# zacz08/ADM

Hardware: AMD Instinct MI355X
Metric: train images/sec (CIFAR-10 32x32 uncond DDM UNet, 1 optimizer step/iter) + 10-step sample images/sec (higher is better)
Workload: dtype f32; 1 GPU; BASELINE configs[1]: CIFAR-10 32x32 uncond two-decoder DhariwalUNet (216M params), bs=128/GPU fp32, ddm_const schedule, dropout 0.1, loss_simple (LPIPS term needs unfetchable VGG16 weights), clip 1.0 + AdamW + EMA(every 8); global_batch=128, image=3x32x32, parallelism=dp1, valid=True

## Files before the change

adm_amd/csrc/conv_wino2d_x6.hip:

```cpp
#include "common.h"
#include "../../include/adm_hip.h"
#include <type_traits>

#ifndef X6_TL
#define X6_TL 0
#endif
#ifndef X6_SHARE
#define X6_SHARE 0
#endif
#ifndef X6_ABL
#define X6_ABL 0
#endif

namespace {

struct X6P {
  const float* x; const unsigned short* w; const float* bias; const float* res; float* y;
  int Mt, N, H, W, Hh, Wh, Cin, ldx, ldy, ldr, wrows, tilesN, xbytes, wbytes, plane;
  int splitk, chunks_per_split; float* ws;
  int ybytes, rbytes;
  int up;
  const float* amax_x; float wscale;
};

typedef __attribute__((address_space(3))) void x6_lds_void;
typedef __bf16 bf16x8 __attribute__((ext_vector_type(8)));
typedef unsigned u32x2 __attribute__((ext_vector_type(2)));
typedef unsigned u32x4 __attribute__((ext_vector_type(4)));
constexpr int X6P_T = 64, X6N = 64, X6K = 16;
[[maybe_unused]] constexpr int X6_A_STAGE = 4 * 3 * X6P_T * X6K;
[[maybe_unused]] constexpr int X6_B_STAGE = 4 * 3 * X6N * X6K;
typedef _Float16 f16x8 __attribute__((ext_vector_type(8)));
typedef _Float16 f16x2 __attribute__((ext_vector_type(2)));
template <int FMT, int NB = 2> struct X6Fmt {
  static constexpr int TERMS = FMT ? 2 : 3;
  static constexpr int NT = 32 * NB;
  static constexpr int CONS = 2 * NB;
  static constexpr int THREADS = (CONS + 4) * 64;
  static constexpr int A_STAGE = 4 * TERMS * X6P_T * X6K;
  static constexpr int B_STAGE = 4 * TERMS * NT * X6K;
  static constexpr int DMA_PER_WAVE = 2 * TERMS;
  static constexpr int RB = NB > 2 ? 3 : 4;
  static constexpr int PD = NB > 2 ? 3 : 4;
};
__device__ __host__ inline float h3_scale(float amax) {
  if (!(amax > 0.f) || !(amax < 3e38f)) return 1.f;
  int e;
  frexpf(16000.f / amax, &e);
  return ldexpf(1.f, e - 1);
}
constexpr int X6_RA = 2;

__device__ __forceinline__ void x6_barrier() {
  __builtin_amdgcn_fence(__ATOMIC_RELEASE, "workgroup", "local");
  __builtin_amdgcn_s_barrier();
// ... 50 lines not shown

__device__ __forceinline__ void x6_store(const f32x4 (&e)[4], unsigned short* la) {
  if (X6_ABL & 2) return;
  const f32x4 v[4] = {p_sub4(e[0], e[2]), p_add4(e[1], e[2]), p_sub4(e[2], e[1]), p_sub4(e[1], e[3])};
#pragma unroll
  for (int ex = 0; ex < 4; ++ex) {
    u32x2 t0, t1, t2;
    split3_pack(v[ex], t0, t1, t2);
    *reinterpret_cast<u32x2*>(la + (ex * 3 + 0) * X6P_T * X6K) = t0;
    *reinterpret_cast<u32x2*>(la + (ex * 3 + 1) * X6P_T * X6K) = t1;
    *reinterpret_cast<u32x2*>(la + (ex * 3 + 2) * X6P_T * X6K) = t2;
  }
}

#ifndef X6_KB_N
#define X6_KB_N 4
#endif
constexpr int X6_KB = X6_KB_N;
struct X6Seq {
  int k0, len, ey, cc, skip2;
  __device__ __forceinline__ void init(int chunks, int up) { k0 = 0; len = min(X6_KB, chunks); ey = 0; cc = 0; skip2 = up; }
  __device__ __forceinline__ int chunk() const { return k0 + cc; }
  __device__ __forceinline__ bool done() const { return len <= 0; }
  __device__ __forceinline__ void next(int chunks) {
    if (++cc == len) {
      cc = 0;
      ++ey;
      if (skip2 && ey == 2) ++ey;
      if (ey == 4) { ey = 0; k0 += len; len = min(X6_KB, chunks - k0); }
    }
  }
};

template <int FMT, int NB>
__global__ __launch_bounds__((2 * NB + 4) * 64) void wino2d_x6_kernel(X6P p) {
  using F = X6Fmt<FMT, NB>;
  constexpr int TERMS = F::TERMS;
  float sa = 1.f, inv_scale = 1.f;
  if (FMT) { sa = h3_scale(adm_amax_read(p.amax_x)); inv_scale = 1.f / (sa * p.wscale); }
  extern __shared__ __attribute__((aligned(16))) unsigned short smem6[];
  unsigned short* As = smem6;
  unsigned short* Bs = smem6 + X6_RA * F::A_STAGE;
  const int tid = threadIdx.x, lane = tid & 63, hw_wid = tid >> 6;
  const bool producer = hw_wid >= F::CONS;
  const int wid = producer ? hw_wid - F::CONS : hw_wid;
  int bid = blockIdx.x;
  {
    const int nwg = gridDim.x, q = nwg >> 3, r = nwg & 7, xcd = bid & 7, idx = bid >> 3;
    bid = (xcd < r ? xcd * (q + 1) : r * (q + 1) + (xcd - r) * q) + idx;
  }
  const int tilesM = gridDim.x / p.tilesN;
  const int tm = bid % tilesM, tn = bid / tilesM;
  const int mt0 = tm * X6P_T, n0 = tn * F::NT;
  constexpr unsigned OOB = 0x80000000u;

  const int c_begin = (p.splitk > 1) ? (int)blockIdx.y * p.chunks_per_split : 0;
  const int chunks = (p.splitk > 1) ? min(p.chunks_per_split, (p.Cin >> 4) - c_begin) : (p.Cin >> 4);
  const int S = (p.up ? 3 : 4) * chunks;

  if (producer) {
    const __amdgpu_buffer_rsrc_t rs_x = __builtin_amdgcn_make_buffer_rsrc(const_cast<float*>(p.x), 0, p.xbytes, 0x00020000);
    const int ptid = wid * 64 + lane;
    const int pl = ptid >> 2, aq = ptid & 3;
    unsigned a_base = 0, colmask = 0, rowmask = 0;
    bool take_l = false, take_r = false;
    {
      const int t = mt0 + pl;
      if (t < p.Mt) {
        const int xp = t % p.Wh;
        const int u = t / p.Wh;
        const int ty = u % p.Hh, b = u / p.Hh;
        a_base = p.up ? (unsigned)((((long)b * p.Hh + ty) * p.Wh + xp) * p.ldx + aq * 4) * 4u
                      : (unsigned)((((long)b * p.H + 2 * ty) * p.W + 2 * xp) * p.ldx + aq * 4) * 4u;
        colmask = (xp > 0 ? 1u : 0u) | 6u | (2 * xp + 2 < p.W ? 8u : 0u);
        rowmask = (ty > 0 ? 1u : 0u) | 6u | (2 * ty + 2 < p.H ? 8u : 0u);
        if (X6_SHARE && !p.up) {
          take_l = xp > 0 && (pl & 15) != 0;
          take_r = xp + 1 < p.Wh && (pl & 15) != 15 && t + 1 < p.Mt;
          if (take_l) colmask &= ~1u;
          if (take_r) colmask &= ~8u;
        }
      }
    }
    unsigned short* la = As + pl * X6K + ((((aq >> 1) ^ (pl >> 3)) & 1) << 3) + (aq & 1) * 4;
    X6Seq ld; ld.init(chunks, p.up);
    unsigned a_voff[2][4];
    int voff_ey = -1;
    auto set_rows = [&]() {
      const int ey = ld.ey;
      const int iA = (ey == 0) ? 0 : 1, iB = (ey == 3) ? 3 : 2;
      const bool live = !ld.done();
      const bool vA = ((rowmask >> iA) & 1u) && live, vB = ((rowmask >> iB) & 1u) && live;
      const int offA = (p.up ? ((iA + 1) >> 1) - 1 : iA - 1) * (p.up ? p.Wh : p.W) * p.ldx * 4;
      const int offB = (p.up ? ((iB + 1) >> 1) - 1 : iB - 1) * (p.up ? p.Wh : p.W) * p.ldx * 4;
#pragma unroll
      for (int j = 0; j < 4; ++j) {
// ... 20 lines not shown
      if (!ld.done()) ld.next(chunks);
    };
    auto store = [&](int d, int slot) {
      f32x4 e[4];
      if (set_ey[d] == 1) {
#pragma unroll
        for (int j = 0; j < 4; ++j) e[j] = p_add4(dA[d][j], dB[d][j]);
      } else if (set_ey[d] == 2) {
#pragma unroll
        for (int j = 0; j < 4; ++j) e[j] = p_sub4(dB[d][j], dA[d][j]);
      } else {
#pragma unroll
        for (int j = 0; j < 4; ++j) e[j] = p_sub4(dA[d][j], dB[d][j]);
      }
      if (X6_SHARE && !p.up) {
        f32x4 el, er;
#pragma unroll
        for (int i = 0; i < 4; ++i) { el[i] = __shfl_up(e[2][i], 4, 64); er[i] = __shfl_down(e[1][i], 4, 64); }
        if (take_l) e[0] = el;
        if (take_r) e[3] = er;
      }
      if (FMT) h3_store(e, la + slot * F::A_STAGE, sa);
      else x6_store(e, la + slot * F::A_STAGE);
    };
#pragma unroll
    for (int d = 0; d < D; ++d) issue(d);
    __builtin_amdgcn_sched_barrier(0);
    constexpr int TRIP = (D & 1) ? 2 * D : D;
    for (int t = 0; t < S; t += TRIP) {
#pragma unroll
      for (int k = 0; k < TRIP; ++k) {
        const int d = k % D;
        if (t + k < S) {
          const bool tl = X6_TL && p.ws && blockIdx.x == 0 && tid == F::CONS * 64 && t + k < 48;
          unsigned long long* TL = reinterpret_cast<unsigned long long*>(p.ws) + 1024 + (t + k) * 4;
          if (tl) TL[0] = __builtin_readcyclecounter();
          store(d, k & 1);
          __builtin_amdgcn_sched_barrier(0);
          if (tl) { asm volatile("s_waitcnt lgkmcnt(0)" ::: "memory"); TL[1] = __builtin_readcyclecounter(); }
          issue(d);
          __builtin_amdgcn_sched_barrier(0);
          if (tl) TL[2] = __builtin_readcyclecounter();
          x6_barrier();
          if (tl) TL[3] = __builtin_readcyclecounter();
        }
      }
    }
    return;
  }

  const __amdgpu_buffer_rsrc_t rs_w = __builtin_amdgcn_make_buffer_rsrc(const_cast<unsigned short*>(p.w), 0, p.wbytes, 0x00020000);
  const int wm = wid / NB, wn = wid % NB;
  const int lr = lane & 31, lh = lane >> 5;
  if (p.splitk > 1) {
    p.y = p.ws + (long)blockIdx.y * ((long)p.Mt * 4) * p.N;
    p.ldy = p.N; p.bias = nullptr; p.res = nullptr;
    const long sb = (long)p.Mt * 4 * p.N * 4;
    p.ybytes = sb < (1L << 31) ? (int)sb : 0;
  }
  constexpr int QW = F::DMA_PER_WAVE;
  unsigned b_voff[QW];
#pragma unroll
  for (int i = 0; i < QW; ++i) {
    const int q = wid * QW + i, pt = q / NB;
    const int row = (q % NB) * 32 + (lane >> 1);
    const int n = n0 + row;
    const int half = (lane ^ (row >> 3)) & 1;
    b_voff[i] = (n < p.wrows) ? (unsigned)((((long)pt * p.wrows + n) * 16 + half * 8) * 2) : OOB;
  }
  X6Seq lb; lb.init(chunks, p.up);
  int ld_slot = 0;
  auto issue_b = [&]() {
    const int kb = ((lb.ey * (p.Cin >> 4) + c_begin + lb.chunk()) * (4 * TERMS) * p.wrows) << 5;
    unsigned short* dst = Bs + ld_slot * F::B_STAGE + (wid * QW) * 512;
    if (!(X6_ABL & 4)) {
#pragma unroll
      for (int i = 0; i < QW; ++i)
        __builtin_amdgcn_raw_ptr_buffer_load_lds(rs_w, (x6_lds_void*)(dst + i * 512), 16, (int)b_voff[i], kb, 0, 0);
    }
    lb.next(chunks);
    if (++ld_slot == F::RB) ld_slot = 0;
  };

  f32x16 acc[4];
  f32x16 Y[2][2];
#pragma unroll
  for (int a = 0; a < 2; ++a)
#pragma unroll
    for (int b = 0; b < 2; ++b)
#pragma unroll
      for (int r = 0; r < 16; ++r) Y[a][b][r] = 0.f;
  const int a_foff = (wm * 32 + lr) * X6K + ((lh ^ (lr >> 3)) & 1) * 8;
  const int b_foff = (wn * 32 + lr) * X6K + ((lh ^ (lr >> 3)) & 1) * 8;
  const f32x16 zero = {0.f, 0.f, 0.f, 0.f, 0.f, 0.f, 0.f, 0.f, 0.f, 0.f, 0.f, 0.f, 0.f, 0.f, 0.f, 0.f};

  X6Seq cs; cs.init(chunks, p.up);
  int slot_b = 0;
#pragma unroll
  for (int i = 0; i < F::RB - 1; ++i) issue_b();
  for (int t = 0; t < S; ++t) {
    const bool tl = X6_TL && p.ws && blockIdx.x == 0 && tid == 0 && t < 48;
    unsigned long long* TL = reinterpret_cast<unsigned long long*>(p.ws) + t * 4;
    if (tl) TL[0] = __builtin_readcyclecounter();
    if (F::RB == 4 && t + 2 < S) { if (FMT) asm volatile("s_waitcnt vmcnt(8) lgkmcnt(0)\n\ts_barrier" ::: "memory"); else asm volatile("s_waitcnt vmcnt(12) lgkmcnt(0)\n\ts_barrier" ::: "memory"); }
    else if (t + 1 < S) { if (FMT) asm volatile("s_waitcnt vmcnt(4) lgkmcnt(0)\n\ts_barrier" ::: "memory"); else asm volatile("s_waitcnt vmcnt(6) lgkmcnt(0)\n\ts_barrier" ::: "memory"); }
    else asm volatile("s_waitcnt vmcnt(0) lgkmcnt(0)\n\ts_barrier" ::: "memory");
    if (tl) TL[1] = __builtin_readcyclecounter();
    if (t + F::RB - 1 < S) issue_b();
    const unsigned short* Ab = As + (t & 1) * F::A_STAGE + a_foff;
    const unsigned short* Bb = Bs + slot_b * F::B_STAGE + b_foff;
    if (++slot_b == F::RB) slot_b = 0;
    const bool first = cs.cc == 0;
    u32x4 fa[NB > 2 ? 1 : 2][TERMS], fb[NB > 2 ? 1 : 2][TERMS];
    auto frag = [&](int xi, int set) {
#pragma unroll
      for (int k = 0; k < TERMS; ++k) {
        if (X6_ABL & 16) {
          fa[set][k] = u32x4{0x3f803f80u, (unsigned)t, 0x3f803f80u, (unsigned)xi};
          fb[set][k] = u32x4{0x3f003f00u, (unsigned)k, 0x3f003f00u, (unsigned)lane};
          continue;
        }
        fa[set][k] = *reinterpret_cast<const u32x4*>(Ab + (xi * TERMS + k) * X6P_T * X6K);
        fb[set][k] = *reinterpret_cast<const u32x4*>(Bb + (xi * TERMS + k) * F::NT * X6K);
      }
    };
    auto products = [&](auto first_tag) {
      if (NB > 2) {
#pragma unroll
        for (int xi = 0; xi < 4; ++xi) {
          frag(xi, 0);
          if (X6_ABL & 8) continue;
          const f16x8 a0 = __builtin_bit_cast(f16x8, fa[0][0]), a1 = __builtin_bit_cast(f16x8, fa[0][1]);
          const f16x8 b0 = __builtin_bit_cast(f16x8, fb[0][0]), b1 = __builtin_bit_cast(f16x8, fb[0][1]);
          f32x16 c;
          if (decltype(first_tag)::value) asm volatile("v_mfma_f32_32x32x16_f16 %0, %1, %2, 0" : "=&v"(c) : "v"(a0), "v"(b1));
          else c = __builtin_amdgcn_mfma_f32_32x32x16_f16(a0, b1, acc[xi], 0, 0, 0);
          c = __builtin_amdgcn_mfma_f32_32x32x16_f16(a1, b0, c, 0, 0, 0);
          acc[xi] = __builtin_amdgcn_mfma_f32_32x32x16_f16(a0, b0, c, 0, 0, 0);
        }
        return;
// ... 9 lines not shown
        if (FMT) {
          const f16x8 a0 = __builtin_bit_cast(f16x8, fa[cur][0]), a1 = __builtin_bit_cast(f16x8, fa[cur][1]);
          const f16x8 b0 = __builtin_bit_cast(f16x8, fb[cur][0]), b1 = __builtin_bit_cast(f16x8, fb[cur][1]);
          f32x16 c = __builtin_amdgcn_mfma_f32_32x32x16_f16(a0, b1, c0, 0, 0, 0);
          c = __builtin_amdgcn_mfma_f32_32x32x16_f16(a1, b0, c, 0, 0, 0);
          acc[xi] = __builtin_amdgcn_mfma_f32_32x32x16_f16(a0, b0, c, 0, 0, 0);
        } else {
          bf16x8 a[3], b[3];
#pragma unroll
          for (int k = 0; k < 3; ++k) { a[k] = __builtin_bit_cast(bf16x8, fa[cur][k % TERMS]); b[k] = __builtin_bit_cast(bf16x8, fb[cur][k % TERMS]); }
          f32x16 c = __builtin_amdgcn_mfma_f32_32x32x16_bf16(a[0], b[2], c0, 0, 0, 0);
          c = __builtin_amdgcn_mfma_f32_32x32x16_bf16(a[2], b[0], c, 0, 0, 0);
          c = __builtin_amdgcn_mfma_f32_32x32x16_bf16(a[1], b[1], c, 0, 0, 0);
          c = __builtin_amdgcn_mfma_f32_32x32x16_bf16(a[0], b[1], c, 0, 0, 0);
          c = __builtin_amdgcn_mfma_f32_32x32x16_bf16(a[1], b[0], c, 0, 0, 0);
          acc[xi] = __builtin_amdgcn_mfma_f32_32x32x16_bf16(a[0], b[0], c, 0, 0, 0);
        }
        __builtin_amdgcn_sched_barrier(0);
      }
    };
    if (first) products(std::true_type{});
    else products(std::false_type{});
    if (tl) TL[2] = __builtin_readcyclecounter();
    const int ey = cs.ey;
    const bool last = cs.cc + 1 == cs.len;
    cs.next(chunks);
    if (last) {
      const f32x16 z0 = acc[0] + acc[1] + acc[2], z1 = sub16(sub16(acc[1], acc[2]), acc[3]);
      if (ey <= 2) { Y[0][0] += z0; Y[0][1] += z1; }
      if (ey == 1) { Y[1][0] += z0; Y[1][1] += z1; }
      if (ey >= 2) { Y[1][0] = sub16(Y[1][0], z0); Y[1][1] = sub16(Y[1][1], z1); }
    }
  }

  const int n = n0 + wn * 32 + lr;
  const float bv = (p.bias && n < p.N) ? p.bias[n] : 0.f;
  const int tb = mt0 + wm * 32 + 4 * lh;
  if (p.ybytes > 0) {
    const __amdgpu_buffer_rsrc_t rs_y = __builtin_amdgcn_make_buffer_rsrc(p.y, 0, p.ybytes, 0x00020000);
    const __amdgpu_buffer_rsrc_t rs_r = __builtin_amdgcn_make_buffer_rsrc(const_cast<float*>(p.res), 0, p.res ? p.rbytes : 0, 0x00020000);
#pragma unroll
    for (int r = 0; r < 16; ++r) {
      const int t = tb + (r & 3) + 8 * (r >> 2);
      const bool ok = t < p.Mt && n < p.N;
      const int xp = t % p.Wh;
      const int u = t / p.Wh;
      const unsigned px0 = ((unsigned)u * 2u) * (unsigned)p.W + 2u * (unsigned)xp;
      unsigned oy[2][2], orr[2][2];
      float rv[2][2];
#pragma unroll
      for (int a = 0; a < 2; ++a)
#pragma unroll
        for (int c = 0; c < 2; ++c) {
          const unsigned px = px0 + (unsigned)a * (unsigned)p.W + (unsigned)c;
          oy[a][c] = ok ? (px * (unsigned)p.ldy + (unsigned)n) * 4u : OOB;
          orr[a][c] = ok ? (px * (unsigned)p.ldr + (unsigned)n) * 4u : OOB;
          rv[a][c] = __builtin_bit_cast(float, __builtin_amdgcn_raw_buffer_load_b32(rs_r, (int)orr[a][c], 0, 0));
        }
#pragma unroll
      for (int a = 0; a < 2; ++a)
#pragma unroll
        for (int c = 0; c < 2; ++c)
          __builtin_amdgcn_raw_buffer_store_b32(__builtin_bit_cast(unsigned, (FMT ? Y[a][c][r] * inv_scale : Y[a][c][r]) + bv + rv[a][c]), rs_y, (int)oy[a][c], 0, 0);
    }
    return;
  }
  if (n >= p.N) return;
#pragma unroll
  for (int r = 0; r < 16; ++r) {
    const int t = tb + (r & 3) + 8 * (r >> 2);
    if (t >= p.Mt) continue;
    const int xp = t % p.Wh;
    const int u = t / p.Wh;
    const long px0 = ((long)u * 2) * p.W + 2 * xp;
#pragma unroll
    for (int a = 0; a < 2; ++a) {
      const long px = px0 + (long)a * p.W;
      float y0 = (FMT ? Y[a][0][r] * inv_scale : Y[a][0][r]) + bv, y1 = (FMT ? Y[a][1][r] * inv_scale : Y[a][1][r]) + bv;
      if (p.res) { y0 += p.res[px * p.ldr + n]; y1 += p.res[(px + 1) * p.ldr + n]; }
      p.y[px * p.ldy + n] = y0;
      p.y[(px + 1) * p.ldy + n] = y1;
    }
  }
}

__global__ void split3_kernel(const float* __restrict__ src, unsigned short* __restrict__ dst, int rows, int cols) {
  const long per = (long)rows * cols, total = per * 16;
  const int chunks = cols >> 4;
  for (long i = blockIdx.x * (long)blockDim.x + threadIdx.x; i < total; i += (long)gridDim.x * blockDim.x) {
    const int img = (int)(i / per);
    const long rc = i - img * per;
    const int n = (int)(rc / cols), c = (int)(rc - (long)n * cols);
    const int ey = img >> 2, ex = img & 3;
    const float a = src[i];
    const unsigned u = __float_as_uint(a);
    const float r = a - __uint_as_float(u & 0xFFFF0000u);
    const unsigned m = __float_as_uint(r);
    const float r2 = r - __uint_as_float(m & 0xFFFF0000u);
    unsigned short* d = dst + ((((long)(ey * chunks + (c >> 4)) * 12 + ex * 3) * rows + n) << 4) + (c & 15);
    const long term = (long)rows << 4;
    d[0] = (unsigned short)(u >> 16);
    d[term] = (unsigned short)(m >> 16);
    d[2 * term] = (unsigned short)(__float_as_uint(r2) >> 16);
  }
}

__global__ void split2_kernel(const float* __restrict__ src, unsigned short* __restrict__ dst, int rows, int cols, float scale,
                              int* __restrict__ overflow) {
  const long per = (long)rows * cols, total = per * 16;
  const int chunks = cols >> 4;
  bool bad = false;
  for (long i = blockIdx.x * (long)blockDim.x + threadIdx.x; i < total; i += (long)gridDim.x * blockDim.x) {
    const int img = (int)(i / per);
    const long rc = i - img * per;
    const int n = (int)(rc / cols), c = (int)(rc - (long)n * cols);
// ... 3 lines not shown
    const _Float16 h0 = (_Float16)a, h1 = (_Float16)(a - (float)h0);
    unsigned short* d = dst + ((((long)(ey * chunks + (c >> 4)) * 8 + ex * 2) * rows + n) << 4) + (c & 15);
    d[0] = __builtin_bit_cast(unsigned short, h0);
    d[(long)rows << 4] = __builtin_bit_cast(unsigned short, h1);
  }
  if (bad && overflow) *overflow = 1;
}

}

int adm_splitk_reduce(const float* ws, const float* bias, const float* res, float* y, long M, int N, int ldy, int ldr, int splitk,
                      hipStream_t stream);

extern "C" int adm_split3_bf16(const float* src, void* dst, int rows, int cols, hipStream_t stream) {
  if (!src || !dst || rows <= 0 || cols <= 0 || (cols & 15)) return ADM_EINVAL;
  const long total = (long)rows * cols * 16;
  const int grid = (int)((total + 255) / 256 > 4096 ? 4096 : (total + 255) / 256);
  hipLaunchKernelGGL(split3_kernel, dim3(grid), dim3(256), 0, stream, src, static_cast<unsigned short*>(dst), rows, cols);
  ADM_CHECK_LAUNCH();
  return ADM_OK;
}

extern "C" int adm_split2_f16(const float* src, void* dst, int rows, int cols, float scale, int* overflow, hipStream_t stream) {
  if (!src || !dst || rows <= 0 || cols <= 0 || (cols & 15) || !(scale > 0.f)) return ADM_EINVAL;
  const long total = (long)rows * cols * 16;
  const int grid = (int)((total + 255) / 256 > 4096 ? 4096 : (total + 255) / 256);
  hipLaunchKernelGGL(split2_kernel, dim3(grid), dim3(256), 0, stream, src, static_cast<unsigned short*>(dst), rows, cols, scale, overflow);
  ADM_CHECK_LAUNCH();
  return ADM_OK;
}

static int g_h3_wide = -1;
extern "C" int adm_wino2d_h3_wide(int v) { const int old = g_h3_wide; g_h3_wide = v; return old; }

static int wino2d_x6_launch(const float* x, const void* wq6, const float* bias, const float* res, float* y, float* ws, long ws_floats,
                            int B, int H, int W, int Cin, int ldx, int N, int wrows, int ldy, int ldr, int up, hipStream_t stream,
                            const float* amax_x = nullptr, float wscale = 0.f) {
  const bool h3 = amax_x != nullptr;
  if (!x || !wq6 || !y || B <= 0 || H < 2 || W < 2 || (W & 1) || (H & 1)) return ADM_EINVAL;
  if ((Cin & 31) || (ldx & 3) || N <= 0 || wrows < N) return ADM_EINVAL;
  if (((uintptr_t)x | (uintptr_t)wq6) & 15) return ADM_EINVAL;
  X6P p;
  p.x = x; p.w = static_cast<const unsigned short*>(wq6); p.bias = bias; p.res = res; p.y = y;
  const long Mt = (long)B * (H / 2) * (W / 2);
  const long xb = (long)B * H * W * ldx * 4 / (up ? 4 : 1), wb = (h3 ? 32L : 48L) * wrows * Cin * 2;
  if (h3 && !(wscale > 0.f)) return ADM_EINVAL;
  if (Mt >= (1L << 30) || xb >= (1L << 31) || wb >= (1L << 31)) return ADM_EINVAL;
  p.Mt = (int)Mt; p.N = N; p.H = H; p.W = W; p.Hh = H / 2; p.Wh = W / 2; p.Cin = Cin; p.ldx = ldx; p.ldy = ldy; p.ldr = ldr;
  p.wrows = wrows; p.xbytes = (int)xb; p.wbytes = (int)wb; p.plane = wrows * Cin; p.up = up ? 1 : 0;
  p.amax_x = amax_x; p.wscale = wscale;
  p.tilesN = adm_cdiv(N, X6N);
  const long mtiles = adm_cdiv(Mt, X6P_T);
  p.splitk = 1; p.chunks_per_split = 0; p.ws = X6_TL ? ws : nullptr;
  const long yb = (long)B * H * W * ldy * 4, rb = res ? (long)B * H * W * ldr * 4 : 0;
  p.ybytes = (yb < (1L << 31) && rb < (1L << 31)) ? (int)yb : 0;
  p.rbytes = (int)rb;
  const int sk = (ws && !(N & 3) && !(ldy & 3) && (!res || !(ldr & 3))) ? adm_wino2d_x6_splitk(B, H, W, Cin, N) : 1;
  if (sk > 1 && ws_floats >= (long)sk * Mt * 4 * N) {
    const int chunks = Cin >> 4;
    p.chunks_per_split = ((chunks + sk - 1) / sk + 1) & ~1;
    p.splitk = (chunks + p.chunks_per_split - 1) / p.chunks_per_split;
    p.ws = ws;
  }
  constexpr int smem0 = (X6_RA * X6Fmt<0>::A_STAGE + X6Fmt<0>::RB * X6Fmt<0>::B_STAGE) * (int)sizeof(unsigned short);
  constexpr int smem1 = (X6_RA * X6Fmt<1>::A_STAGE + X6Fmt<1>::RB * X6Fmt<1>::B_STAGE) * (int)sizeof(unsigned short);
  constexpr int smemw = (X6_RA * X6Fmt<1, 4>::A_STAGE + X6Fmt<1, 4>::RB * X6Fmt<1, 4>::B_STAGE) * (int)sizeof(unsigned short);
  constexpr int smem3 = (X6_RA * X6Fmt<1, 3>::A_STAGE + X6Fmt<1, 3>::RB * X6Fmt<1, 3>::B_STAGE) * (int)sizeof(unsigned short);
  static bool attr_set = false;
  if (!attr_set) {
    if (hipFuncSetAttribute(reinterpret_cast<const void*>(&wino2d_x6_kernel<0, 2>), hipFuncAttributeMaxDynamicSharedMemorySize, smem0) != hipSuccess ||
        hipFuncSetAttribute(reinterpret_cast<const void*>(&wino2d_x6_kernel<1, 2>), hipFuncAttributeMaxDynamicSharedMemorySize, smem1) != hipSuccess ||
        hipFuncSetAttribute(reinterpret_cast<const void*>(&wino2d_x6_kernel<1, 4>), hipFuncAttributeMaxDynamicSharedMemorySize, smemw) != hipSuccess ||
        hipFuncSetAttribute(reinterpret_cast<const void*>(&wino2d_x6_kernel<1, 3>), hipFuncAttributeMaxDynamicSharedMemorySize, smem3) != hipSuccess)
      return ADM_ELAUNCH;
    attr_set = true;
  }
  int form = 2;
  if (h3 && p.splitk == 1 && g_h3_wide != 0 && N > X6N) {
    if (g_h3_wide == 1) form = 4;
    else if (g_h3_wide == 3) form = 3;
    else {
      const long cost[3] = {48, 60, 64};
      long best = -1;
      for (int nb = 2; nb <= 4; ++nb) {
        const long t = (mtiles * adm_cdiv(N, 32 * nb) + 255) / 256 * cost[nb - 2];
        if (best < 0 || t < best) { best = t; form = nb; }
      }
    }
  }
  const bool three = form == 3, wide = form == 4;
  if (three) {
    p.tilesN = adm_cdiv(N, X6Fmt<1, 3>::NT);
    hipLaunchKernelGGL((wino2d_x6_kernel<1, 3>), dim3((unsigned)(mtiles * p.tilesN), 1), dim3(X6Fmt<1, 3>::THREADS), smem3, stream, p);
  } else if (wide) {
    p.tilesN = adm_cdiv(N, X6Fmt<1, 4>::NT);
    hipLaunchKernelGGL((wino2d_x6_kernel<1, 4>), dim3((unsigned)(mtiles * p.tilesN), 1), dim3(X6Fmt<1, 4>::THREADS), smemw, stream, p);
  } else if (h3) {
    hipLaunchKernelGGL((wino2d_x6_kernel<1, 2>), dim3((unsigned)(mtiles * p.tilesN), p.splitk), dim3(512), smem1, stream, p);
  } else {
    hipLaunchKernelGGL((wino2d_x6_kernel<0, 2>), dim3((unsigned)(mtiles * p.tilesN), p.splitk), dim3(512), smem0, stream, p);
  }
  ADM_CHECK_LAUNCH();
  if (p.splitk > 1) return adm_splitk_reduce(ws, bias, res, y, Mt * 4, N, ldy, ldr, p.splitk, stream);
  return ADM_OK;
}

extern "C" int adm_conv_fwd_wino2d_h3(const float* x, const void* wqh, const float* bias, const float* res, float* y, float* ws,
                                      long ws_floats, int B, int H, int W, int Cin, int ldx, int N, int wrows, int ldy, int ldr,
                                      const float* amax_x, float wscale, int up, hipStream_t stream) {
  if (!amax_x) return ADM_EINVAL;
  return wino2d_x6_launch(x, wqh, bias, res, y, ws, ws_floats, B, H, W, Cin, ldx, N, wrows, ldy, ldr, up, stream, amax_x, wscale);
}

extern "C" int adm_conv_fwd_wino2d_x6(const float* x, const void* wq6, const float* bias, const float* res, float* y, float* ws,
                                      long ws_floats, int B, int H, int W, int Cin, int ldx, int N, int wrows, int ldy, int ldr,
                                      hipStream_t stream) {
  return wino2d_x6_launch(x, wq6, bias, res, y, ws, ws_floats, B, H, W, Cin, ldx, N, wrows, ldy, ldr, 0, stream);
}

extern "C" int adm_conv_fwd_wino2d_x6_up(const float* x, const void* wq6, const float* bias, const float* res, float* y, float* ws,
                                         long ws_floats, int B, int H, int W, int Cin, int ldx, int N, int wrows, int ldy, int ldr,
                                         hipStream_t stream) {
  return wino2d_x6_launch(x, wq6, bias, res, y, ws, ws_floats, B, H, W, Cin, ldx, N, wrows, ldy, ldr, 1, stream);
}

extern "C" int adm_wino2d_x6_splitk(int B, int H, int W, int Cin, int N) {
  const long wgs = (long)adm_cdiv((long)B * (H / 2) * (W / 2), X6P_T) * adm_cdiv(N, X6N);
  const int chunks = Cin >> 4;
// ... 12 lines not shown
```

adm_amd/hip.py:

```python
from __future__ import annotations

import ctypes
import os
import subprocess
from ctypes import c_double, c_float, c_int, c_long, c_uint64, c_void_p

import torch

_HERE = os.path.dirname(os.path.abspath(__file__))
LIB_PATH = os.path.join(_HERE, "libadm_hip.so")
_lib = None

P, I, L, F, D, U = c_void_p, c_int, c_long, c_float, c_double, c_uint64
_SIGS = {
    "adm_version": [],
    "adm_conv_fwd": [P, P, P, P, P, I, I, I, I, I, I, I, I, I, I, I, I, P],
    "adm_conv_splitk": [I, I, I],
    "adm_conv_fwd_ws": [P, P, P, P, P, P, L, I, I, I, I, I, I, I, I, I, I, I, P],
    "adm_conv_fwd_strided": [P, P, P, P, P, I, I, I, I, I, I, I, I, I, I, I, I, I, I, P],
    "adm_conv_fwd_wino": [P, P, P, P, P, I, I, I, I, I, I, I, I, I, P],
    "adm_conv_fwd_wino_up": [P, P, P, P, P, I, I, I, I, I, I, I, I, I, P],
    "adm_pack_weight_wino": [P, P, P, I, I, I, I, P],
    "adm_pack_weight_wino2d": [P, P, P, I, I, I, I, P],
    "adm_conv_fwd_wino2d": [P, P, P, P, P, P, L, I, I, I, I, I, I, I, I, I, P],
    "adm_wino2d_splitk": [I, I, I, I, I],
    "adm_wino2d_variant": [I],
    "adm_wino2d_h3_wide": [I],
    "adm_wgrad_h3_blocks": [I],
    "adm_conv_fwd_wino2d_x6": [P, P, P, P, P, P, L, I, I, I, I, I, I, I, I, I, P],
    "adm_conv_fwd_wino2d_x6_up": [P, P, P, P, P, P, L, I, I, I, I, I, I, I, I, I, P],
    "adm_wino2d_x6_splitk": [I, I, I, I, I],
    "adm_split3_bf16": [P, P, I, I, P],
    "adm_split2_f16": [P, P, I, I, F, P, P],
    "adm_conv_fwd_wino2d_h3": [P, P, P, P, P, P, L, I, I, I, I, I, I, I, I, I, P, F, I, P],
    "adm_gemm_x6": [P, P, P, P, P, L, I, I, I, I, I, I, P],
    "adm_gemm_x6_amax": [P, P, P, P, P, L, I, I, I, I, I, I, P, P],
    "adm_gemm_x6_h3": [P, P, P, P, P, L, I, I, I, I, I, I, P, F, P, P],
    "adm_split2_rows_f16": [P, P, I, I, I, F, P, P],
    "adm_split3_rows": [P, P, I, I, I, P],
    "adm_conv_wgrad_x6": [P, P, P, P, I, I, I, I, I, I, I, I, P],
    "adm_conv_wgrad_x6_up": [P, P, P, P, I, I, I, I, I, I, I, I, P],
    "adm_conv_wgrad_x6_ws": [P, P, P, P, I, I, I, I, I, I, I, I, I, P],
    "adm_conv_wgrad_x6_plan": [I, I, I, I, I],
    "adm_gemm_wgrad_x6": [P, P, P, P, L, I, I, I, I, I, P],
    "adm_gemm_wgrad_x6_ws": [P, P, P, P, L, I, I, I, I, I, P],
    "adm_gemm_wgrad_x6_plan": [L, I, I],
    "adm_conv_wgrad_x6_h3": [P, P, P, P, I, I, I, I, I, I, I, I, I, I, P, P, P],
    "adm_gemm_wgrad_x6_h3": [P, P, P, P, L, I, I, I, I, I, I, P, P, P],
    "adm_conv_wgrad_x6_bf16a": [P, P, P, P, I, I, I, I, I, I, I, I, I, P],
    "adm_gemm_wgrad_x6_bf16a": [P, P, P, P, L, I, I, I, I, I, P],
    "adm_conv_wgrad": [P, P, P, I, I, I, I, I, I, I, I, I, I, P],
    "adm_conv_wgrad_wino": [P, P, P, P, I, I, I, I, I, I, I, I, P],
    "adm_conv_wgrad_wino_up": [P, P, P, P, I, I, I, I, I, I, I, I, P],
    "adm_conv_wgrad_bias": [P, P, P, P, I, I, I, I, I, I, I, I, I, I, P],
    "adm_conv_wgrad_wino2d": [P, P, P, P, I, I, I, I, I, I, I, I, P],
    "adm_unpack_wgrad_wino2d": [P, I, P, I, I, I, I, I, P, P, P],
    "adm_conv_wgrad_plan": [I, I, I, I, I, I, I, I],
    "adm_conv_wgrad_ws": [P, P, P, P, I, I, I, I, I, I, I, I, I, I, I, P],
    "adm_unpack_wgrad_splits": [P, I, P, I, I, I, I, I, I, I, P, P, P],
    "adm_conv_fwd_bf16": [P, P, P, P, P, I, I, I, I, I, I, I, I, I, I, I, I, P],
# ... 97 lines not shown
    "adm_logit_terms_bwd": [P, I, I, P, F, P, L, P],
    "adm_leaky_relu_fwd": [P, P, L, F, P],
    "adm_leaky_relu_bwd": [P, P, P, L, F, P],
    "adm_softmax_rows_bwd": [P, P, L, I, L, F, P],
    "adm_transpose2d": [P, P, I, I, P],
    "adm_adaptive_weight": [P, L, P, L, P, F, P, P],
    "adm_axpy_dev": [P, P, P, F, P, L, P],
}
EXPORTS = tuple(_SIGS)


def build(verbose: bool = False) -> str:
    r = subprocess.run(["make", "-C", os.path.join(_HERE, "csrc"), "-j8"], capture_output=True, text=True)
    if verbose or r.returncode != 0:
        print(r.stdout[-4000:], r.stderr[-8000:])
    if r.returncode != 0 or not os.path.exists(LIB_PATH):
        raise RuntimeError("building libadm_hip.so failed")
    return LIB_PATH


def lib() -> ctypes.CDLL:
    global _lib
    if _lib is None:
        if not os.path.exists(LIB_PATH):
            raise RuntimeError(f"{LIB_PATH} is missing: run `python -c 'import __graft_entry__ as g; g.build()'` "
                               "(there is no non-HIP fallback for the adm_amd hot path)")
        _lib = ctypes.CDLL(LIB_PATH)
        for name, args in _SIGS.items():
            fn = getattr(_lib, name)
            fn.argtypes = args
            fn.restype = c_long if name in ("adm_aug_workspace_floats", "adm_linattn_ws_floats") else c_int
        if os.environ.get("ADM_H3_WIDE") is not None:
            _lib.adm_wino2d_h3_wide(int(os.environ["ADM_H3_WIDE"]))
        if os.environ.get("ADM_WGRAD_H3_BLOCKS") is not None:
            _lib.adm_wgrad_h3_blocks(int(os.environ["ADM_WGRAD_H3_BLOCKS"]))
    return _lib


def stream() -> c_void_p:
    return c_void_p(torch.cuda.current_stream().cuda_stream)


def ptr(t) -> c_void_p:
    return None if t is None else c_void_p(t.data_ptr())


NO_STREAM = ("adm_version", "adm_conv_splitk", "adm_gn_splits", "adm_aug_workspace_floats", "adm_conv_wgrad_plan",
             "adm_sumsq_blocks", "adm_lnc_blocks", "adm_bn_blocks", "adm_linattn_ws_floats", "adm_wino2d_splitk", "adm_wino2d_x6_splitk", "adm_wino2d_variant", "adm_wino2d_h3_wide", "adm_wgrad_h3_blocks", "adm_gn_fused", "adm_conv_wgrad_x6_plan", "adm_gemm_wgrad_x6_plan", "adm_lpips_head_blocks", "adm_ae_blocks")


def call(name: str, *args):
    rc = getattr(lib(), name)(*args, stream())
    if rc != 0:
        raise RuntimeError(f"{name} failed with code {rc} (-22 = unsupported shape/alignment, -5 = launch failure)")


def require_cuda(t: torch.Tensor, what: str = "tensor"):
    if not t.is_cuda:
        raise RuntimeError(f"adm_amd: {what} is on {t.device}; the HIP hot path needs a GPU tensor "
                           "(no CPU fallback exists by design)")
```

include/adm_hip.h:

```cpp
#ifndef ADM_HIP_H
#define ADM_HIP_H
#include <stdint.h>
typedef struct ihipStream_t* hipStream_t;

#ifdef __cplusplus
#define ADM_AMAX_SLOTS 64
#define ADM_AMAX_STRIDE 32
#define ADM_AMAX_FLOATS (ADM_AMAX_SLOTS * ADM_AMAX_STRIDE)

extern "C" {
#endif

int adm_version(void);


int adm_conv_fwd(const float* x, const float* wp, const float* bias, const float* res, float* y,
                 int B, int H, int W, int Cin, int ldx, int N, int wrows, int ldy, int ldr,
                 int ks, int up, int tile, hipStream_t stream);

int adm_conv_fwd_strided(const float* x, const float* wp, const float* bias, const float* res, float* y,
                         int B, int Hin, int Win, int Hout, int Wout, int Cin, int ldx, int N, int wrows,
                         int ldy, int ldr, int ks, int stride, int pad_lo, hipStream_t stream);

int adm_conv_fwd_wino(const float* x, const float* wq, const float* bias, const float* res, float* y, int B, int H, int W,
// ... 34 lines not shown
                           long ws_floats, int B, int H, int W, int Cin, int ldx, int N, int wrows, int ldy, int ldr,
                           const float* amax_x, float wscale, int up, hipStream_t stream);
int adm_split3_bf16(const float* src, void* dst, int rows, int cols, hipStream_t stream);
int adm_gemm_x6(const float* x, const void* w6, const float* bias, const float* res, float* y, long M, int K, int ldx, int N, int wrows,
                int ldy, int ldr, hipStream_t stream);
int adm_split3_rows(const float* src, void* dst, int rows, int cols, int ld, hipStream_t stream);
int adm_gemm_x6_amax(const float* x, const void* w6, const float* bias, const float* res, float* y, long M, int K, int ldx, int N,
                     int wrows, int ldy, int ldr, float* amax_y, hipStream_t stream);
int adm_gemm_x6_h3(const float* x, const void* wh, const float* bias, const float* res, float* y, long M, int K, int ldx, int N, int wrows,
                   int ldy, int ldr, const float* amax_x, float wscale, float* amax_y, hipStream_t stream);
int adm_split2_rows_f16(const float* src, void* dst, int rows, int cols, int ld, float scale, int* overflow, hipStream_t stream);
int adm_conv_wgrad_x6(const float* x, const float* dy, float* dwp2, float* dbias, int B, int H, int W, int Cin, int ldx, int Cout,
                      int lddy, int splits, hipStream_t stream);
int adm_conv_wgrad_x6_up(const float* x, const float* dy, float* dwp2, float* dbias, int B, int H, int W, int Cin, int ldx, int Cout,
                         int lddy, int splits, hipStream_t stream);
int adm_conv_wgrad_x6_ws(const float* x, const float* dy, float* ws, float* bws, int B, int H, int W, int Cin, int ldx, int Cout,
                         int lddy, int splits, int up, hipStream_t stream);
int adm_conv_wgrad_x6_plan(int B, int H, int W, int Cin, int Cout);
int adm_gemm_wgrad_x6(const float* x, const float* dy, float* dwp, float* dbias, long P, int Cin, int ldx, int Cout, int lddy,
                      int splits, hipStream_t stream);
int adm_gemm_wgrad_x6_ws(const float* x, const float* dy, float* ws, float* bws, long P, int Cin, int ldx, int Cout, int lddy,
                         int splits, hipStream_t stream);
int adm_gemm_wgrad_x6_plan(long P, int Cin, int Cout);
int adm_conv_wgrad_x6_bf16a(const void* x16, const float* dy, float* dwp2, float* dbias, int B, int H, int W, int Cin, int ldx,
                            int Cout, int lddy, int splits, int up, hipStream_t stream);
int adm_gemm_wgrad_x6_bf16a(const void* x16, const float* dy, float* dwp, float* dbias, long P, int Cin, int ldx, int Cout, int lddy,
                            int splits, hipStream_t stream);
int adm_conv_wgrad_x6_h3(const float* x, const float* dy, float* dwp2, float* dbias, int B, int H, int W, int Cin, int ldx, int Cout,
                         int lddy, int splits, int up, int det, const float* amax_x, const float* amax_dy, hipStream_t stream);
int adm_gemm_wgrad_x6_h3(const float* x, const float* dy, float* dwp, float* dbias, long P, int Cin, int ldx, int Cout, int lddy,
                         int splits, int det, const float* amax_x, const float* amax_dy, hipStream_t stream);
int adm_wino2d_variant(int ws);
int adm_wino2d_h3_wide(int v);
int adm_wgrad_h3_blocks(int v);
int adm_wino2d_splitk(int B, int H, int W, int Cin, int N);

int adm_conv_wgrad_wino2d(const float* x, const float* dy, float* dwp2, float* dbias, int B, int H, int W, int Cin, int ldx,
                          int Cout, int lddy, int splits, hipStream_t stream);
int adm_unpack_wgrad_wino2d(const float* wx, int splits, float* dw, int Co, int Ci, int Co_pad, int Ci_pad, int accumulate,
                            const float* bws, float* dbias, hipStream_t stream);

int adm_conv_wgrad_plan(int B, int H, int W, int Cin, int Cout, int ks, int up, int wino);
int adm_conv_wgrad_ws(const float* x, const float* dy, float* ws, float* bws, int B, int H, int W, int Cin, int ldx, int Cout,
                      int lddy, int ks, int up, int splits, int wino, hipStream_t stream);

int adm_conv_fwd_bf16(const float* x, const unsigned short* wp16, const float* bias, const float* res, float* y,
                      int B, int H, int W, int Cin, int ldx, int N, int wrows, int ldy, int ldr, int ks, int up,
                      int tile, hipStream_t stream);
int adm_conv_wgrad_bf16(const float* x, const float* dy, float* dwp, int B, int H, int W, int Cin, int ldx, int Cout,
                        int lddy, int ks, int up, int splits, hipStream_t stream);
int adm_conv_fwd_bf16a(const void* x16, const unsigned short* wp16, const float* bias, const float* res, float* y, int B, int H, int W,
                       int Cin, int ldx, int N, int wrows, int ldy, int ldr, int ks, int up, int tile, hipStream_t stream);
int adm_conv_wgrad_bf16a(const void* x16, const float* dy, float* dwp, int B, int H, int W, int Cin, int ldx, int Cout, int lddy, int ks,
                         int up, int splits, hipStream_t stream);
int adm_gn_fwd_bf16out(const float* x, float* stats, double* ws, const float* gamma, const float* beta, const float* ss,
                       long ss_bstride, void* y16, int B, int HW, int C, int G, float eps, int silu, float drop_p, uint64_t seed,
                       hipStream_t stream);
int adm_f32_to_bf16(const float* src, unsigned short* dst, long n, hipStream_t stream);

int adm_pack_weight(const float* w, float* wp_fwd, float* wp_bwd, int Co, int Ci, int ks, int Co_pad, int Ci_pad,
                    int qkv, hipStream_t stream);
int adm_pack_weight_table(const long* table, int n_entries, long total_tiles, hipStream_t stream);
int adm_unpack_wgrad(const float* dwp, float* dw, int Co, int Ci, int ks, int Co_pad, int Ci_pad, int qkv,
                     int accumulate, hipStream_t stream);
int adm_unpack_wgrad_splits(const float* ws, int splits, float* dw, int Co, int Ci, int ks, int Co_pad, int Ci_pad, int qkv,
                            int accumulate, const float* bws, float* dbias, hipStream_t stream);
// ... 211 lines not shown
```

Measured before the change: 1241 images/s.

## Make Winograd x6 h3 conv kernel persistent with prefetch across tiles

Adds a persistent-grid variant of the Winograd x6 forward conv kernel for the h3 path without split-K, enabled by default when the tile count exceeds the CU count. Each workgroup loops over tiles, and consumers issue the next tile's weight loads before writing the current tile's epilogue, so loads overlap with stores and launch/tail costs shrink. Weight load offsets are now computed per issue from a scalar base rather than held in per-lane precomputed registers. This adds a drain barrier and extra control flow, and the grid is limited to one workgroup per CU, which may reduce occupancy.

```diff
diff --git a/adm_amd/csrc/conv_wino2d_x6.hip b/adm_amd/csrc/conv_wino2d_x6.hip
--- a/adm_amd/csrc/conv_wino2d_x6.hip
+++ b/adm_amd/csrc/conv_wino2d_x6.hip
@@ -21,6 +21,7 @@
   int ybytes, rbytes;
   int up;
   const float* amax_x; float wscale;
+  int ntiles;
 };
 
 typedef __attribute__((address_space(3))) void x6_lds_void;
@@ -137,26 +138,29 @@
   }
 };
 
-template <int FMT, int NB>
+template <int FMT, int NB, bool PS = false>
 __global__ __launch_bounds__((2 * NB + 4) * 64) void wino2d_x6_kernel(X6P p) {
   using F = X6Fmt<FMT, NB>;
   constexpr int TERMS = F::TERMS;
-  float sa = 1.f, inv_scale = 1.f;
-  if (FMT) { sa = h3_scale(adm_amax_read(p.amax_x)); inv_scale = 1.f / (sa * p.wscale); }
+  float sa = 1.f;
+  if (FMT) sa = h3_scale(adm_amax_read(p.amax_x));
+  const int sa_bits = __builtin_amdgcn_readfirstlane(__builtin_bit_cast(int, sa));
   extern __shared__ __attribute__((aligned(16))) unsigned short smem6[];
   unsigned short* As = smem6;
   unsigned short* Bs = smem6 + X6_RA * F::A_STAGE;
   const int tid = threadIdx.x, lane = tid & 63, hw_wid = tid >> 6;
   const bool producer = hw_wid >= F::CONS;
   const int wid = producer ? hw_wid - F::CONS : hw_wid;
-  int bid = blockIdx.x;
-  {
-    const int nwg = gridDim.x, q = nwg >> 3, r = nwg & 7, xcd = bid & 7, idx = bid >> 3;
-    bid = (xcd < r ? xcd * (q + 1) : r * (q + 1) + (xcd - r) * q) + idx;
-  }
-  const int tilesM = gridDim.x / p.tilesN;
-  const int tm = bid % tilesM, tn = bid / tilesM;
-  const int mt0 = tm * X6P_T, n0 = tn * F::NT;
+  const int nwg = PS ? p.ntiles : (int)gridDim.x, G = gridDim.x;
+  int L = blockIdx.x;
+  auto tile_of = [&](int l, int& mt0_, int& n0_) {
+    const int q = nwg >> 3, r = nwg & 7, xcd = l & 7, idx = l >> 3;
+    const int bid = (xcd < r ? xcd * (q + 1) : r * (q + 1) + (xcd - r) * q) + idx;
+    const int tilesM = nwg / p.tilesN;
+    mt0_ = (bid % tilesM) * X6P_T; n0_ = (bid / tilesM) * F::NT;
+  };
+  int mt0, n0;
+  tile_of(L, mt0, n0);
   constexpr unsigned OOB = 0x80000000u;
 
   const int c_begin = (p.splitk > 1) ? (int)blockIdx.y * p.chunks_per_split : 0;
@@ -167,6 +171,7 @@
     const __amdgpu_buffer_rsrc_t rs_x = __builtin_amdgcn_make_buffer_rsrc(const_cast<float*>(p.x), 0, p.xbytes, 0x00020000);
     const int ptid = wid * 64 + lane;
     const int pl = ptid >> 2, aq = ptid & 3;
+    for (;;) {
     unsigned a_base = 0, colmask = 0, rowmask = 0;
     bool take_l = false, take_r = false;
     {
@@ -253,7 +258,7 @@
       for (int k = 0; k < TRIP; ++k) {
         const int d = k % D;
         if (t + k < S) {
-          const bool tl = X6_TL && p.ws && blockIdx.x == 0 && tid == F::CONS * 64 && t + k < 48;
+          const bool tl = X6_TL && p.ws && L == 0 && tid == F::CONS * 64 && t + k < 48;
           unsigned long long* TL = reinterpret_cast<unsigned long long*>(p.ws) + 1024 + (t + k) * 4;
           if (tl) TL[0] = __builtin_readcyclecounter();
           store(d, k & 1);
@@ -267,7 +272,9 @@
         }
       }
     }
-    return;
+    if (!PS || (L += G) >= nwg) return;
+    tile_of(L, mt0, n0);
+    }
   }
 
   const __amdgpu_buffer_rsrc_t rs_w = __builtin_amdgcn_make_buffer_rsrc(const_cast<unsigned short*>(p.w), 0, p.wbytes, 0x00020000);
@@ -280,24 +287,22 @@
     p.ybytes = sb < (1L << 31) ? (int)sb : 0;
   }
   constexpr int QW = F::DMA_PER_WAVE;
-  unsigned b_voff[QW];
-#pragma unroll
-  for (int i = 0; i < QW; ++i) {
-    const int q = wid * QW + i, pt = q / NB;
-    const int row = (q % NB) * 32 + (lane >> 1);
-    const int n = n0 + row;
-    const int half = (lane ^ (row >> 3)) & 1;
-    b_voff[i] = (n < p.wrows) ? (unsigned)((((long)pt * p.wrows + n) * 16 + half * 8) * 2) : OOB;
-  }
+  const int swid = __builtin_amdgcn_readfirstlane(wid);
+  const unsigned b_lane = (unsigned)((lane >> 1) * 32 + ((lane ^ (lane >> 4)) & 1) * 16);
+  int n0_b = n0;
   X6Seq lb; lb.init(chunks, p.up);
   int ld_slot = 0;
   auto issue_b = [&]() {
     const int kb = ((lb.ey * (p.Cin >> 4) + c_begin + lb.chunk()) * (4 * TERMS) * p.wrows) << 5;
-    unsigned short* dst = Bs + ld_slot * F::B_STAGE + (wid * QW) * 512;
+    unsigned short* dst = Bs + ld_slot * F::B_STAGE + (swid * QW) * 512;
     if (!(X6_ABL & 4)) {
 #pragma unroll
-      for (int i = 0; i < QW; ++i)
-        __builtin_amdgcn_raw_ptr_buffer_load_lds(rs_w, (x6_lds_void*)(dst + i * 512), 16, (int)b_voff[i], kb, 0, 0);
+      for (int i = 0; i < QW; ++i) {
+        const int q = swid * QW + i, pt = q / NB, nb = n0_b + (q % NB) * 32;
+        const unsigned voff = (int)(b_lane >> 5) < p.wrows - nb ? b_lane : OOB;
+        const int soff = kb + (nb < p.wrows ? (pt * p.wrows + nb) << 5 : 0);
+        __builtin_amdgcn_raw_ptr_buffer_load_lds(rs_w, (x6_lds_void*)(dst + i * 512), 16, (int)voff, soff, 0, 0);
+      }
     }
     lb.next(chunks);
     if (++ld_slot == F::RB) ld_slot = 0;
@@ -305,28 +310,39 @@
 
   f32x16 acc[4];
   f32x16 Y[2][2];
-#pragma unroll
-  for (int a = 0; a < 2; ++a)
-#pragma unroll
-    for (int b = 0; b < 2; ++b)
-#pragma unroll
-      for (int r = 0; r < 16; ++r) Y[a][b][r] = 0.f;
   const int a_foff = (wm * 32 + lr) * X6K + ((lh ^ (lr >> 3)) & 1) * 8;
   const int b_foff = (wn * 32 + lr) * X6K + ((lh ^ (lr >> 3)) & 1) * 8;
   const f32x16 zero = {0.f, 0.f, 0.f, 0.f, 0.f, 0.f, 0.f, 0.f, 0.f, 0.f, 0.f, 0.f, 0.f, 0.f, 0.f, 0.f};
 
-  X6Seq cs; cs.init(chunks, p.up);
+  X6Seq cs;
   int slot_b = 0;
+  bool drain = false;
+  const bool tl0 = X6_TL && p.ws && blockIdx.x == 0 && tid == 0;
+  unsigned long long* TLB = reinterpret_cast<unsigned long long*>(p.ws) + 2048;
+  if (tl0) TLB[0] = __builtin_readcyclecounter();
 #pragma unroll
   for (int i = 0; i < F::RB - 1; ++i) issue_b();
+  for (;;) {
+  float y0 = 0.f;
+  if (PS) asm volatile("" : "+v"(y0));
+#pragma unroll
+  for (int a = 0; a < 2; ++a)
+#pragma unroll
+    for (int b = 0; b < 2; ++b)
+#pragma unroll
+      for (int r = 0; r < 16; ++r) Y[a][b][r] = y0;
+  cs.init(chunks, p.up);
+#pragma clang loop unroll(disable)
   for (int t = 0; t < S; ++t) {
-    const bool tl = X6_TL && p.ws && blockIdx.x == 0 && tid == 0 && t < 48;
+    const bool tl = X6_TL && p.ws && L == 0 && tid == 0 && t < 48;
     unsigned long long* TL = reinterpret_cast<unsigned long long*>(p.ws) + t * 4;
     if (tl) TL[0] = __builtin_readcyclecounter();
-    if (F::RB == 4 && t + 2 < S) { if (FMT) asm volatile("s_waitcnt vmcnt(8) lgkmcnt(0)\n\ts_barrier" ::: "memory"); else asm volatile("s_waitcnt vmcnt(12) lgkmcnt(0)\n\ts_barrier" ::: "memory"); }
+    if (PS && drain && t == 0) asm volatile("s_waitcnt vmcnt(0) lgkmcnt(0)\n\ts_barrier" ::: "memory");
+    else if (F::RB == 4 && t + 2 < S) { if (FMT) asm volatile("s_waitcnt vmcnt(8) lgkmcnt(0)\n\ts_barrier" ::: "memory"); else asm volatile("s_waitcnt vmcnt(12) lgkmcnt(0)\n\ts_barrier" ::: "memory"); }
     else if (t + 1 < S) { if (FMT) asm volatile("s_waitcnt vmcnt(4) lgkmcnt(0)\n\ts_barrier" ::: "memory"); else asm volatile("s_waitcnt vmcnt(6) lgkmcnt(0)\n\ts_barrier" ::: "memory"); }
     else asm volatile("s_waitcnt vmcnt(0) lgkmcnt(0)\n\ts_barrier" ::: "memory");
     if (tl) TL[1] = __builtin_readcyclecounter();
+    if (tl0 && t == 0 && (!drain || L == G)) TLB[drain ? 5 : 1] = __builtin_readcyclecounter();
     if (t + F::RB - 1 < S) issue_b();
     const unsigned short* Ab = As + (t & 1) * F::A_STAGE + a_foff;
     const unsigned short* Bb = Bs + slot_b * F::B_STAGE + b_foff;
@@ -402,10 +418,25 @@
       if (ey >= 2) { Y[1][0] = sub16(Y[1][0], z0); Y[1][1] = sub16(Y[1][1], z1); }
     }
   }
-
-  const int n = n0 + wn * 32 + lr;
+  const bool tlb = tl0 && !drain;
+  if (tlb) TLB[2] = __builtin_readcyclecounter();
+  int btid = tid, bWh = p.Wh, bsa = sa_bits;
+  if (PS) asm volatile("" : "+v"(btid), "+s"(bWh), "+s"(bsa));
+  const float inv_scale = FMT ? 1.f / (__builtin_bit_cast(float, bsa) * p.wscale) : 1.f;
+  const int blane = btid & 63, bwid = btid >> 6;
+  const bool more = PS && L + G < nwg;
+  int mt0_next = 0, n0_next = 0;
+  if (more) {
+    tile_of(L + G, mt0_next, n0_next);
+    n0_b = n0_next;
+    lb.init(chunks, p.up);
+#pragma unroll
+    for (int i = 0; i < F::RB - 1; ++i) issue_b();
+  }
+
+  const int n = n0 + (bwid % NB) * 32 + (blane & 31);
   const float bv = (p.bias && n < p.N) ? p.bias[n] : 0.f;
-  const int tb = mt0 + wm * 32 + 4 * lh;
+  const int tb = mt0 + (bwid / NB) * 32 + 4 * (blane >> 5);
   if (p.ybytes > 0) {
     const __amdgpu_buffer_rsrc_t rs_y = __builtin_amdgcn_make_buffer_rsrc(p.y, 0, p.ybytes, 0x00020000);
     const __amdgpu_buffer_rsrc_t rs_r = __builtin_amdgcn_make_buffer_rsrc(const_cast<float*>(p.res), 0, p.res ? p.rbytes : 0, 0x00020000);
@@ -413,8 +444,8 @@
     for (int r = 0; r < 16; ++r) {
       const int t = tb + (r & 3) + 8 * (r >> 2);
       const bool ok = t < p.Mt && n < p.N;
-      const int xp = t % p.Wh;
-      const int u = t / p.Wh;
+      const int xp = t % bWh;
+      const int u = t / bWh;
       const unsigned px0 = ((unsigned)u * 2u) * (unsigned)p.W + 2u * (unsigned)xp;
       unsigned oy[2][2], orr[2][2];
       float rv[2][2];
@@ -433,15 +464,13 @@
         for (int c = 0; c < 2; ++c)
           __builtin_amdgcn_raw_buffer_store_b32(__builtin_bit_cast(unsigned, (FMT ? Y[a][c][r] * inv_scale : Y[a][c][r]) + bv + rv[a][c]), rs_y, (int)oy[a][c], 0, 0);
     }
-    return;
-  }
-  if (n >= p.N) return;
+  } else if (n < p.N) {
 #pragma unroll
   for (int r = 0; r < 16; ++r) {
     const int t = tb + (r & 3) + 8 * (r >> 2);
     if (t >= p.Mt) continue;
-    const int xp = t % p.Wh;
-    const int u = t / p.Wh;
+    const int xp = t % bWh;
+    const int u = t / bWh;
     const long px0 = ((long)u * 2) * p.W + 2 * xp;
 #pragma unroll
     for (int a = 0; a < 2; ++a) {
@@ -451,6 +480,15 @@
       p.y[px * p.ldy + n] = y0;
       p.y[(px + 1) * p.ldy + n] = y1;
     }
+  }
+  }
+  if (tlb) {
+    TLB[3] = __builtin_readcyclecounter();
+    asm volatile("s_waitcnt vmcnt(0)" ::: "memory");
+    TLB[4] = __builtin_readcyclecounter();
+  }
+  if (!more) return;
+  L += G; mt0 = mt0_next; n0 = n0_next; drain = true;
   }
 }
 
@@ -520,6 +558,8 @@
 
 static int g_h3_wide = -1;
 extern "C" int adm_wino2d_h3_wide(int v) { const int old = g_h3_wide; g_h3_wide = v; return old; }
+static int g_x6_persist = -1;
+extern "C" int adm_wino2d_x6_persist(int v) { const int old = g_x6_persist; g_x6_persist = v; return old; }
 
 static int wino2d_x6_launch(const float* x, const void* wq6, const float* bias, const float* res, float* y, float* ws, long ws_floats,
                             int B, int H, int W, int Cin, int ldx, int N, int wrows, int ldy, int ldr, int up, hipStream_t stream,
@@ -555,7 +595,16 @@
   constexpr int smemw = (X6_RA * X6Fmt<1, 4>::A_STAGE + X6Fmt<1, 4>::RB * X6Fmt<1, 4>::B_STAGE) * (int)sizeof(unsigned short);
   constexpr int smem3 = (X6_RA * X6Fmt<1, 3>::A_STAGE + X6Fmt<1, 3>::RB * X6Fmt<1, 3>::B_STAGE) * (int)sizeof(unsigned short);
   static bool attr_set = false;
+  static int cus = 0;
   if (!attr_set) {
+    int dev = 0;
+    hipDeviceProp_t prop;
+    if (hipGetDevice(&dev) != hipSuccess || hipGetDeviceProperties(&prop, dev) != hipSuccess || prop.multiProcessorCount <= 0) return ADM_ELAUNCH;
+    cus = prop.multiProcessorCount;
+    if (hipFuncSetAttribute(reinterpret_cast<const void*>(&wino2d_x6_kernel<1, 2, true>), hipFuncAttributeMaxDynamicSharedMemorySize, smem1) != hipSuccess ||
+        hipFuncSetAttribute(reinterpret_cast<const void*>(&wino2d_x6_kernel<1, 4, true>), hipFuncAttributeMaxDynamicSharedMemorySize, smemw) != hipSuccess ||
+        hipFuncSetAttribute(reinterpret_cast<const void*>(&wino2d_x6_kernel<1, 3, true>), hipFuncAttributeMaxDynamicSharedMemorySize, smem3) != hipSuccess)
+      return ADM_ELAUNCH;
     if (hipFuncSetAttribute(reinterpret_cast<const void*>(&wino2d_x6_kernel<0, 2>), hipFuncAttributeMaxDynamicSharedMemorySize, smem0) != hipSuccess ||
         hipFuncSetAttribute(reinterpret_cast<const void*>(&wino2d_x6_kernel<1, 2>), hipFuncAttributeMaxDynamicSharedMemorySize, smem1) != hipSuccess ||
         hipFuncSetAttribute(reinterpret_cast<const void*>(&wino2d_x6_kernel<1, 4>), hipFuncAttributeMaxDynamicSharedMemorySize, smemw) != hipSuccess ||
@@ -577,11 +626,22 @@
     }
   }
   const bool three = form == 3, wide = form == 4;
-  if (three) {
-    p.tilesN = adm_cdiv(N, X6Fmt<1, 3>::NT);
+  if (three) p.tilesN = adm_cdiv(N, X6Fmt<1, 3>::NT);
+  if (wide) p.tilesN = adm_cdiv(N, X6Fmt<1, 4>::NT);
+  const long tiles = mtiles * p.tilesN;
+  p.ntiles = (int)tiles;
+  long pg = 0;
+  if (h3 && p.splitk == 1 && g_x6_persist != 0) {
+    if (g_x6_persist > 0) pg = tiles < g_x6_persist ? tiles : g_x6_persist;
+    else if (tiles > cus) pg = cus;
+  }
+  if (pg > 0) {
+    if (three) hipLaunchKernelGGL((wino2d_x6_kernel<1, 3, true>), dim3((unsigned)pg, 1), dim3(X6Fmt<1, 3>::THREADS), smem3, stream, p);
+    else if (wide) hipLaunchKernelGGL((wino2d_x6_kernel<1, 4, true>), dim3((unsigned)pg, 1), dim3(X6Fmt<1, 4>::THREADS), smemw, stream, p);
+    else hipLaunchKernelGGL((wino2d_x6_kernel<1, 2, true>), dim3((unsigned)pg, 1), dim3(512), smem1, stream, p);
+  } else if (three) {
     hipLaunchKernelGGL((wino2d_x6_kernel<1, 3>), dim3((unsigned)(mtiles * p.tilesN), 1), dim3(X6Fmt<1, 3>::THREADS), smem3, stream, p);
   } else if (wide) {
-    p.tilesN = adm_cdiv(N, X6Fmt<1, 4>::NT);
     hipLaunchKernelGGL((wino2d_x6_kernel<1, 4>), dim3((unsigned)(mtiles * p.tilesN), 1), dim3(X6Fmt<1, 4>::THREADS), smemw, stream, p);
   } else if (h3) {
     hipLaunchKernelGGL((wino2d_x6_kernel<1, 2>), dim3((unsigned)(mtiles * p.tilesN), p.splitk), dim3(512), smem1, stream, p);
diff --git a/adm_amd/hip.py b/adm_amd/hip.py
--- a/adm_amd/hip.py
+++ b/adm_amd/hip.py
@@ -26,6 +26,7 @@
     "adm_wino2d_splitk": [I, I, I, I, I],
     "adm_wino2d_variant": [I],
     "adm_wino2d_h3_wide": [I],
+    "adm_wino2d_x6_persist": [I],
     "adm_wgrad_h3_blocks": [I],
     "adm_conv_fwd_wino2d_x6": [P, P, P, P, P, P, L, I, I, I, I, I, I, I, I, I, P],
     "adm_conv_fwd_wino2d_x6_up": [P, P, P, P, P, P, L, I, I, I, I, I, I, I, I, I, P],
@@ -189,6 +190,8 @@
             fn.restype = c_long if name in ("adm_aug_workspace_floats", "adm_linattn_ws_floats") else c_int
         if os.environ.get("ADM_H3_WIDE") is not None:
             _lib.adm_wino2d_h3_wide(int(os.environ["ADM_H3_WIDE"]))
+        if os.environ.get("ADM_X6_PERSIST") is not None:
+            _lib.adm_wino2d_x6_persist(int(os.environ["ADM_X6_PERSIST"]))
         if os.environ.get("ADM_WGRAD_H3_BLOCKS") is not None:
             _lib.adm_wgrad_h3_blocks(int(os.environ["ADM_WGRAD_H3_BLOCKS"]))
     return _lib
@@ -203,7 +206,7 @@
 
 
 NO_STREAM = ("adm_version", "adm_conv_splitk", "adm_gn_splits", "adm_aug_workspace_floats", "adm_conv_wgrad_plan",
-             "adm_sumsq_blocks", "adm_lnc_blocks", "adm_bn_blocks", "adm_linattn_ws_floats", "adm_wino2d_splitk", "adm_wino2d_x6_splitk", "adm_wino2d_variant", "adm_wino2d_h3_wide", "adm_wgrad_h3_blocks", "adm_gn_fused", "adm_conv_wgrad_x6_plan", "adm_gemm_wgrad_x6_plan", "adm_lpips_head_blocks", "adm_ae_blocks")
+             "adm_sumsq_blocks", "adm_lnc_blocks", "adm_bn_blocks", "adm_linattn_ws_floats", "adm_wino2d_splitk", "adm_wino2d_x6_splitk", "adm_wino2d_variant", "adm_wino2d_h3_wide", "adm_wino2d_x6_persist", "adm_wgrad_h3_blocks", "adm_gn_fused", "adm_conv_wgrad_x6_plan", "adm_gemm_wgrad_x6_plan", "adm_lpips_head_blocks", "adm_ae_blocks")
 
 
 def call(name: str, *args):
diff --git a/include/adm_hip.h b/include/adm_hip.h
--- a/include/adm_hip.h
+++ b/include/adm_hip.h
@@ -90,6 +90,7 @@
                          int splits, int det, const float* amax_x, const float* amax_dy, hipStream_t stream);
 int adm_wino2d_variant(int ws);
 int adm_wino2d_h3_wide(int v);
+int adm_wino2d_x6_persist(int v);
 int adm_wgrad_h3_blocks(int v);
 int adm_wino2d_splitk(int B, int H, int W, int Cin, int N);
 
```

Result: no change. 1250 images/s, median of 6 (+0.7%).
